# ishine/TTS-3

Hardware: AMD Instinct MI355X
Metric: audio samples/sec + RTF, HiFiGAN-v1 22.05kHz 80-mel, batch 32 @ 1/2/4/8 GPU (higher is better)
Workload: dtype fp32 (power-of-2 scaled fp16 hi/lo split on fp16 MFMA, fp32 accumulate); 1 GPU; HiFiGAN-v1 22.05kHz inference, [32,80,1024] mel per GPU (replicate pad 5), fp32; model=HiFiGAN-v1 (hifigan_config.py generator_model_params), global_batch=32, seq_len=1024, parallelism=dp1 (utterance sharding; no collectives)

## Files before the change

### tts-3_amd/csrc/conv_device.hpp

```cpp
#pragma once

#include "common.hpp"

namespace tts {

typedef __amdgpu_buffer_rsrc_t rsrc_t;
typedef unsigned u32x4_t __attribute__((ext_vector_type(4)));
typedef unsigned u32x2_t __attribute__((ext_vector_type(2)));
typedef float f32x2 __attribute__((ext_vector_type(2)));
constexpr unsigned OOB_OFF = 0x80000000u;

#ifndef ACT_ABLATE
#define ACT_ABLATE 0
#endif
__device__ __forceinline__ unsigned act_range(unsigned bytes) {
  return (ACT_ABLATE && bytes != 0xFFFFFFFFu && bytes > 65536u) ? 65536u : bytes;
}
__device__ __forceinline__ rsrc_t make_rsrc(const void* p, unsigned bytes) {
  return __builtin_amdgcn_make_buffer_rsrc(const_cast<void*>(p), (short)0, (int)act_range(bytes), 0x00020000);
}
__device__ __forceinline__ float bload(rsrc_t r, unsigned voff, unsigned soff) {
  return __builtin_bit_cast(float, __builtin_amdgcn_raw_buffer_load_b32(r, (int)voff, (int)soff, 0));
}
__device__ __forceinline__ f32x4 bload4(rsrc_t r, unsigned voff, unsigned soff) {
  return __builtin_bit_cast(f32x4, __builtin_amdgcn_raw_buffer_load_b128(r, (int)voff, (int)soff, 0));
}
#ifndef TTS_ST_POL
#define TTS_ST_POL 0
#endif
#ifndef TTS_LDX_POL
#define TTS_LDX_POL 0
#endif
template <int POL = TTS_LDX_POL>
__device__ __forceinline__ float bload_x(rsrc_t r, unsigned voff, unsigned soff) {
  return __builtin_bit_cast(float, __builtin_amdgcn_raw_buffer_load_b32(r, (int)voff, (int)soff, POL));
}
__device__ __forceinline__ void bstore(rsrc_t r, float v, unsigned voff, unsigned soff) {
  __builtin_amdgcn_raw_buffer_store_b32(__builtin_bit_cast(unsigned, v), r, (int)voff, (int)soff, TTS_ST_POL);
}
__device__ __forceinline__ unsigned short f32_to_bf16_bits(float v) {
  return __builtin_bit_cast(unsigned short, (__bf16)v);
}
__device__ __forceinline__ float bf16_bits_to_f32(unsigned b) { return __builtin_bit_cast(float, b << 16); }
__device__ __forceinline__ float bf16_round(float v) { return bf16_bits_to_f32(f32_to_bf16_bits(v)); }
template <bool B16>
struct PlaneT {
  static constexpr unsigned ES = 4u;
  __device__ static __forceinline__ float ld(rsrc_t r, unsigned voff, unsigned soff) { return bload(r, voff, soff); }
  __device__ static __forceinline__ void st(rsrc_t r, float v, unsigned voff, unsigned soff) { bstore(r, v, voff, soff); }
  __device__ static __forceinline__ float rt(float v) { return v; }
};
template <>
struct PlaneT<true> {
  static constexpr unsigned ES = 2u;
  __device__ static __forceinline__ float ld(rsrc_t r, unsigned voff, unsigned soff) {
    return bf16_bits_to_f32((unsigned)__builtin_amdgcn_raw_buffer_load_b16(r, (int)voff, (int)soff, 0));
  }
  __device__ static __forceinline__ void st(rsrc_t r, float v, unsigned voff, unsigned soff) {
    __builtin_amdgcn_raw_buffer_store_b16(f32_to_bf16_bits(v), r, (int)voff, (int)soff, TTS_ST_POL);
  }
  __device__ static __forceinline__ float rt(float v) { return bf16_round(v); }
};
template <bool B16>
__device__ __forceinline__ const void* plane_at(const float* p, size_t e) {
  return reinterpret_cast<const char*>(p) + e * PlaneT<B16>::ES;
}
template <bool B16>
__device__ __forceinline__ f32x4 pload4(rsrc_t r, unsigned voff, unsigned soff) {
  if constexpr (B16) {
    const u32x2_t w = __builtin_bit_cast(u32x2_t, __builtin_amdgcn_raw_buffer_load_b64(r, (int)voff, (int)soff, 0));
    return f32x4{bf16_bits_to_f32(w[0] & 0xffffu), bf16_bits_to_f32(w[0] >> 16), bf16_bits_to_f32(w[1] & 0xffffu),
                 bf16_bits_to_f32(w[1] >> 16)};
  } else {
    return bload4(r, voff, soff);
  }
}
template <bool B16>
__device__ __forceinline__ void pstore4(rsrc_t r, f32x4 v, unsigned voff, unsigned soff) {
  if constexpr (B16) {
    const u32x2_t w = {(unsigned)f32_to_bf16_bits(v[0]) | ((unsigned)f32_to_bf16_bits(v[1]) << 16),
                       (unsigned)f32_to_bf16_bits(v[2]) | ((unsigned)f32_to_bf16_bits(v[3]) << 16)};
    __builtin_amdgcn_raw_buffer_store_b64(__builtin_bit_cast(u32x2_t, w), r, (int)voff, (int)soff, TTS_ST_POL);
  } else {
    __builtin_amdgcn_raw_buffer_store_b128(__builtin_bit_cast(u32x4_t, v), r, (int)voff, (int)soff, TTS_ST_POL);
  }
}

__device__ __forceinline__ void lds_dma_b128(const void* base, unsigned bytes, unsigned voff, const void* lds) {
  const unsigned long long p = reinterpret_cast<unsigned long long>(base);
  const u32x4_t d = {(unsigned)__builtin_amdgcn_readfirstlane((int)(unsigned)p),
                     (unsigned)__builtin_amdgcn_readfirstlane((int)((unsigned)(p >> 32) & 0xffffu)),
                     (unsigned)__builtin_amdgcn_readfirstlane((int)act_range(bytes)), 0x00020000u};
  const unsigned m =
      (unsigned)__builtin_amdgcn_readfirstlane((int)(unsigned)(unsigned long)(__attribute__((address_space(3))) const void*)lds);
#pragma clang diagnostic push
#pragma clang diagnostic ignored "-Winline-asm"
  asm volatile("s_mov_b32 m0, %2\n\ts_nop 0\n\tbuffer_load_dwordx4 %0, %1, 0 offen lds" ::"v"(voff), "s"(d), "s"(m)
               : "memory", "m0");
#pragma clang diagnostic pop
}

__device__ __forceinline__ void l2_touch_dma(const void* base, unsigned bytes, unsigned voff, const void* lds) {
  const unsigned long long p = reinterpret_cast<unsigned long long>(base);
  const u32x4_t d = {(unsigned)__builtin_amdgcn_readfirstlane((int)(unsigned)p),
                     (unsigned)__builtin_amdgcn_readfirstlane((int)((unsigned)(p >> 32) & 0xffffu)),
                     (unsigned)__builtin_amdgcn_readfirstlane((int)act_range(bytes)), 0x00020000u};
  const unsigned m =
      (unsigned)__builtin_amdgcn_readfirstlane((int)(unsigned)(unsigned long)(__attribute__((address_space(3))) const void*)lds);
#pragma clang diagnostic push
#pragma clang diagnostic ignored "-Winline-asm"
  asm volatile("s_mov_b32 m0, %2\n\ts_nop 0\n\tbuffer_load_dword %0, %1, 0 offen lds" ::"v"(voff), "s"(d), "s"(m)
               : "memory", "m0");
#pragma clang diagnostic pop
}

__device__ __forceinline__ float lrelu2(float x, float slope) { return fmaxf(x, x * slope); }
__device__ __forceinline__ int wave_id() { return __builtin_amdgcn_readfirstlane((int)(threadIdx.x >> 6)); }

__device__ __forceinline__ int xlds_off(int g, int r, int q, int xrows) {
  return (g * xrows + r) * 8 + 4 * (q ^ ((r >> 3) & 1));
}

template <int CTRL, int ROWS>
__device__ __forceinline__ float dpp_max_step(float v) {
  const int o = __builtin_amdgcn_update_dpp(__builtin_bit_cast(int, v), __builtin_bit_cast(int, v), CTRL, ROWS, 0xF, false);
  return fmaxf(v, __builtin_bit_cast(float, o));
}
__device__ __forceinline__ float wave_max(float v) {
  v = dpp_max_step<0xB1, 0xF>(v);
  v = dpp_max_step<0x4E, 0xF>(v);
  v = dpp_max_step<0x141, 0xF>(v);
  v = dpp_max_step<0x140, 0xF>(v);
  v = dpp_max_step<0x142, 0xA>(v);
  v = dpp_max_step<0x143, 0xC>(v);
  return __builtin_bit_cast(float, __builtin_amdgcn_readlane(__builtin_bit_cast(int, v), 63));
}

__device__ __forceinline__ void publish_amax(unsigned* slots, int b, float v) {
  v = wave_max(v);
  if ((threadIdx.x & 63) == 0) atomicMax(slots + (size_t)b * 64 + (blockIdx.x & 63), __float_as_uint(v));
}

__device__ __forceinline__ void publish_amax_block(unsigned* slots, int b, float v) {
  __shared__ float red[4];
  v = wave_max(v);
  if ((threadIdx.x & 63) == 0) red[threadIdx.x >> 6] = v;
  __syncthreads();
  if (threadIdx.x == 0)
    atomicMax(slots + (size_t)b * 64 + (blockIdx.x & 63),
              __float_as_uint(fmaxf(fmaxf(red[0], red[1]), fmaxf(red[2], red[3]))));
}

template <int TM, int TN, bool RES, int ZM, bool AMAX, bool YB = false>
__device__ __forceinline__ void conv_epilogue_impl(const Conv1dArgs& a, const f32x16 (&acc)[TM][TN], int b,
                                                   int tbase, int cobase, int lane, int tend,
                                                   const float* sbias, int sbase) {
  using PY = PlaneT<YB>;
  const int half = lane >> 5;
  const int l32 = lane & 31;
  const int Cout = a.Cout;
  const int Tout = a.Tout;
  const unsigned plane = (unsigned)Cout * (unsigned)Tout * PY::ES;
  const size_t item = (size_t)b * (a.o_bstride ? a.o_bstride : (int64_t)Cout * Tout);
  const rsrc_t rres = make_rsrc(RES ? plane_at<YB>(a.res, item) : a.bias, RES ? plane : 0u);
  const rsrc_t rz = make_rsrc(ZM >= 2 ? plane_at<YB>(a.z, item) : a.bias, ZM >= 2 ? plane : 0u);
  const rsrc_t rout = make_rsrc(plane_at<YB>(a.zmode == 0 ? a.y : a.z, item), plane);
  const rsrc_t rcv = make_rsrc(a.cvec ? a.cvec + (size_t)b * (a.cvec_bstride ? a.cvec_bstride : (int64_t)Cout) : a.bias,
                               a.cvec ? (unsigned)Cout * 4u : 0u);
  const rsrc_t rmask = make_rsrc(a.mask ? a.mask + (size_t)b * Tout : a.bias, a.mask ? (unsigned)Tout * 4u : 0u);
  const rsrc_t rbias = make_rsrc(a.bias, (unsigned)Cout * 4u);
  const bool has_mask = a.mask != nullptr;
  const bool mask_res = RES && a.mask_res && has_mask;
  const float oslope = a.out_slope;
  const float zdiv = a.zdiv;
  const unsigned rowb = (unsigned)Tout * PY::ES;
  float vmax = 0.f;
#pragma unroll
  for (int m = 0; m < TM; ++m) {
    float bv[16];
#pragma unroll
    for (int r = 0; r < 16; ++r) {
      const unsigned co = (unsigned)(cobase + m * 32 + (r & 3) + 8 * (r >> 2) + 4 * half);
      bv[r] = sbias ? sbias[(int)co - sbase] : bload(rbias, co * 4u, 0u) + bload(rcv, co * 4u, 0u);
    }
#pragma unroll
    for (int n = 0; n < TN; ++n) {
      const int t = tbase + n * 32 + l32;
      const int row0 = cobase + m * 32 + 4 * half;
      const bool tok = t < Tout && t < tend;
      const unsigned voff = tok ? ((unsigned)row0 * (unsigned)Tout + (unsigned)t) * PY::ES : OOB_OFF;
      const float mv = has_mask ? bload(rmask, (tok ? (unsigned)t * 4u : OOB_OFF), 0u) : 1.f;
      const float mv2 = mask_res ? mv : 1.f;
      unsigned vo[16];
      float rv[16], zv[16];
// ... 190 lines not shown
```

### tts-3_amd/csrc/wino8_kernel.hpp

```cpp
#pragma once

#include <type_traits>

#include "wino_kernel.hpp"

namespace tts {

__device__ __forceinline__ void lds_sync() { asm volatile("s_waitcnt lgkmcnt(0)\n\ts_barrier" ::: "memory"); }

#ifndef WINO_STAMPS
#define WINO_STAMPS 0
#endif
#define WSTAMP(i)                                                                                            \
  do {                                                                                                       \
    if (WINO_STAMPS && (threadIdx.x & 63) == 0) {                                                            \
      const size_t wg = blockIdx.x + (size_t)gridDim.x * (blockIdx.y + (size_t)gridDim.y * blockIdx.z);      \
      reinterpret_cast<unsigned long long*>(a.z)[(wg * 8 + (threadIdx.x >> 6)) * 32 + (i)] =                   \
          __builtin_amdgcn_s_memtime();                                                                      \
    }                                                                                                        \
  } while (0)

template <class S, int K, int D, bool XB = false>
struct Wino8Cfg {
  static constexpr int ES = XB ? 2 : 4;
  static constexpr int AL = 16 / ES;
  static constexpr int NCH = wino_chunks(K);
  static constexpr int NS = kWinoPoints * NCH;
  static constexpr int PAD = D * (K - 1) / 2;
  static constexpr int BNT = 64;
  static constexpr int J = BNT / D;
  static constexpr int TW = 4 * D * J;
  static constexpr int XROWS = BNT + (NCH - 1) * D;
  static constexpr int PLANE = XROWS * S::ROWB;
  static constexpr int TSZ = kWinoPoints * PLANE;
  static constexpr bool RT_ROFF = XB && TW % 8 != 0;
  static constexpr int ROFF = RT_ROFF ? 7 : (AL - PAD % AL) % AL;
  static constexpr int RSPAN = (XROWS - 1) % D + 4 * D * ((XROWS - 1) / D) + 6 * D + ROFF + 1;
  static constexpr int RSPAN4 = (RSPAN + AL - 1) / AL * AL;
  static constexpr int RPITCH = RSPAN4 % (2 * AL) == AL ? RSPAN4 : RSPAN4 + AL;
  static constexpr int RF4 = (16 * RPITCH / AL + 63) / 64 * 64;
  static constexpr int RSZ = RF4 * 16;
  static constexpr int NDMA = RF4 / 64;
  static constexpr int UNITS = XROWS * 4;
  static constexpr int UPW = (UNITS + 7) / 8;
  static constexpr int PITCH = 256;
  static_assert(UPW <= 64 && UNITS <= 256 + 64 && 3 * NCH >= 3, "one transform round per wave; the DMA spreads over 3 steps");
  static_assert(2 * (UNITS - 256) <= 4 * 64, "spread leftover jobs: one per lane of waves 4-7");
  static_assert(TW <= PITCH, "");
  static constexpr int EPI = 4 * 16 * PITCH * 4 > 8 * 8 * 4 * 64 * 4 ? 4 * 16 * PITCH * 4 : 8 * 8 * 4 * 64 * 4;
  static constexpr int TSM = 2 * TSZ > EPI ? 2 * TSZ : EPI;
};

template <class S, int K, int D, bool LRELU, int PL = 0>
__global__ __launch_bounds__(512) void conv1d_wino8_kernel(Conv1dArgs a) {
  constexpr bool XB = (PL & kPlaneXB16) != 0, YB = (PL & kPlaneYB16) != 0;
  using C = Wino8Cfg<S, K, D, XB>;
  constexpr int NP = S::NP;
  constexpr int NCH = C::NCH;
  constexpr bool H3 = S::SCALED;
  static_assert(PL == 0 || !H3, "bf16 planes: the bf16 scheme only");
#ifndef WINO8_PD
#define WINO8_PD 3
#endif
#ifndef WINO8_EARLY_W
#define WINO8_EARLY_W 0
#endif
#ifndef WINO8_PD1
#define WINO8_PD1 4
#endif
#ifndef WINO8_PD11
#define WINO8_PD11 WINO8_PD
#endif
#ifndef WINO8_PD_B1
#define WINO8_PD_B1 3
#endif
#ifndef WINO8_PD1_B1
#define WINO8_PD1_B1 4
#endif
#ifndef WINO8_GAP7
#define WINO8_GAP7 1
#endif
#ifndef WINO8_GAP11
#define WINO8_GAP11 1
#endif
  __shared__ __attribute__((aligned(16))) unsigned char tsm[C::TSM];
  __shared__ __attribute__((aligned(16))) unsigned char rsm[2 * C::RSZ];
  __shared__ float wbias[128];

  const int tid = threadIdx.x;
  const int lane = tid & 63;
  const int wave = __builtin_amdgcn_readfirstlane(tid >> 6);
  const int wm = wave & 3;
  const int grp = wave >> 2;
  const int half = lane >> 5;
  const int l32 = lane & 31;
  const int bx = blockIdx.x, mt = blockIdx.y, b = blockIdx.z;
  const int t0 = bx * C::TW;
  const int Tin = a.Tin;
  const int Cin = a.Cin;
  const int nc = a.n_chunks;
  const int ex = H3 ? amax_exp(a.amax_in, b) + kWinoBtShift : 0;
  const float xscale = H3 ? ldexpf(1.f, -ex) : 1.f;
  const float slope = a.in_slope;
  const char* xb = static_cast<const char*>(plane_at<XB>(a.x, (size_t)b * (a.x_bstride ? a.x_bstride : (int64_t)Cin * Tin)));
  const unsigned chb = (unsigned)Tin * (unsigned)C::ES;

  const int roff = C::RT_ROFF ? (((t0 - C::PAD) % 8) + 8) % 8 : C::ROFF;
  const int ta = t0 - C::PAD - roff;
#ifndef WINO8_ASM_DMA
#define WINO8_ASM_DMA 1
#endif
  auto dma = [&](int c, int rb, int k0 = 0, int k1 = 64) {
    const int c0 = c * 16;
    const rsrc_t rx = make_rsrc(xb + (size_t)c0 * chb, (unsigned)(Cin - c0) * chb);
    for (int i = wm + 4 * k0; i < C::NDMA && i < wm + 4 * k1; i += 4) {
      const int f = i * 64 + lane;
      constexpr int UPR = C::RPITCH / C::AL;
      const int ch = f / UPR, t = ta + C::AL * (f - ch * UPR);
      const unsigned vo = (ch < 16 && t >= 0 && t < Tin) ? (unsigned)ch * chb + (unsigned)t * (unsigned)C::ES : OOB_OFF;
      if (WINO8_ASM_DMA) {
        lds_dma_b128(xb + (size_t)c0 * chb, (unsigned)(Cin - c0) * chb, vo, rsm + rb * C::RSZ + i * 1024);
      } else {
        __builtin_amdgcn_raw_ptr_buffer_load_lds(
            rx, (__attribute__((address_space(3))) void*)(rsm + rb * C::RSZ + i * 1024), 16, (int)vo, 0, 0, 0);
      }
    }
  };

#ifndef WINO8_DENSE
// ... 25 lines not shown
#ifndef WINO8_REMAT11
#define WINO8_REMAT11 1
#endif
  constexpr bool remat = K == 11 ? WINO8_REMAT11 : WINO8_REMAT;
  auto job_unit = [&](int& jrow, int& jq) {
    if (remat && WINO8_DENSE && grp == TG) {
      int ln;
      asm volatile("v_mbcnt_lo_u32_b32 %0, -1, 0\n\tv_mbcnt_hi_u32_b32 %0, -1, %0" : "=v"(ln));
      const int uu = wm * 64 + ln;
      jrow = uu >> 2;
      jq = uu & 3;
    } else {
      jrow = jrow0;
      jq = jq0;
    }
  };
  auto job_load = [&](int rb, int j) {
    if (SPREAD && grp != TG && j >= 2) return;
    if (!uok) return;
    int jrow, jq;
    job_unit(jrow, jq);
    if constexpr (D == 1 && XB) {
      const u32x2_t* raw8 =
          reinterpret_cast<const u32x2_t*>(rsm + rb * C::RSZ) + (4 * jq + piece(j)) * (C::RPITCH / 4) + jrow;
#pragma unroll
      for (int u4 = 0; u4 < NU; ++u4) jraw8[u4] = raw8[u4];
    } else if constexpr (D == 1) {
      const f32x4* raw4 =
          reinterpret_cast<const f32x4*>(rsm + rb * C::RSZ) + (4 * jq + piece(j)) * (C::RPITCH / 4) + jrow;
#pragma unroll
      for (int u4 = 0; u4 < NU; ++u4) jraw4[u4] = raw4[u4];
    } else if constexpr (XB) {
      const int jjj = jrow / D, jrho = jrow - jjj * D;
      const unsigned short* raw = reinterpret_cast<const unsigned short*>(rsm + rb * C::RSZ) +
                                  (4 * jq + piece(j)) * C::RPITCH + jrho + 4 * D * jjj + roff;
#pragma unroll
      for (int k = 0; k < 7; ++k) jraw[k] = bf16_bits_to_f32(raw[D * k]);
    } else {
      const int jjj = jrow / D, jrho = jrow - jjj * D;
      const float* raw = reinterpret_cast<const float*>(rsm + rb * C::RSZ) + (4 * jq + piece(j)) * C::RPITCH +
                         jrho + 4 * D * jjj + C::ROFF;
#pragma unroll
      for (int k = 0; k < 7; ++k) jraw[k] = raw[D * k];
    }
  };
  auto job_finish = [&](int tb, int j) {
    if (SPREAD && grp != TG && j >= 2) return;
    if (!uok) return;
    int jrow, jq;
    job_unit(jrow, jq);
    float v[7], t[7];
#pragma unroll
    for (int k = 0; k < 7; ++k) {
      float x;
      if constexpr (D == 1 && XB) {
        const unsigned w = jraw8[(C::ROFF + k) / 4][((C::ROFF + k) % 4) / 2];
        x = bf16_bits_to_f32((C::ROFF + k) % 2 ? w >> 16 : w & 0xffffu);
      } else {
        x = D == 1 ? jraw4[(C::ROFF + k) / 4][(C::ROFF + k) % 4] : jraw[k];
      }
      if (LRELU) x = lrelu2(x, slope);
      v[k] = H3 ? x * xscale : x;
    }
    wino_bt(v, t);
    if ((j & 1) == 0) {
#pragma unroll
      for (int k = 0; k < 7; ++k) tkeep[k] = t[k];
      return;
    }
    unsigned char* base = tsm + tb * C::TSZ + jrow * S::ROWB + 4 * jq + 16 * (piece(j) >> 1);
#pragma unroll
    for (int p = 0; p < kWinoPoints; ++p) {
      unsigned w[NP];
      split_pair<S>(tkeep[p], t[p], w);
#pragma unroll
      for (int q = 0; q < NP; ++q) *reinterpret_cast<unsigned*>(base + p * C::PLANE + 32 * q) = w[q];
    }
  };

  const int mb = mt * 4 + wm;
  const rsrc_t ra = make_rsrc(a.w + ((size_t)mb * nc * C::NS) * (NP * 256), 0xFFFFFFFFu);
  const unsigned avoff = (unsigned)lane * 16u;

#ifndef WINO8_NOXCH
#define WINO8_NOXCH 0
#endif
  constexpr bool NX = WINO8_NOXCH != 0;
  constexpr int NA = NX ? 7 : 4, NB = NX ? 1 : 2;
  f32x16 acc[NA][NB];
#pragma unroll
  for (int p = 0; p < NA; ++p)
#pragma unroll
    for (int n = 0; n < NB; ++n) acc[p][n] = f32x16{};
  WSTAMP(0);

  float bpre = 0.f;
  if (tid < 128) {
    const int co = mt * 128 + tid;
    if (co < a.Cout) {
      bpre = a.bias[co];
      const float cv = a.cvec ? a.cvec[(size_t)b * (a.cvec_bstride ? a.cvec_bstride : (int64_t)a.Cout) + co] : 0.f;
      bpre = bpre + cv;
    }
  }
  if (grp == 1) {
    dma(0, 0);
    if (nc > 1) dma(1, 1);
  }
  auto prologue = [&](auto wl_tag) {
    constexpr int WL = decltype(wl_tag)::value;
    if (grp == 1) {
      if (nc > 1) asm volatile("s_waitcnt vmcnt(%0)" ::"n"(C::NDMA / 4 + WL) : "memory");
      else asm volatile("s_waitcnt vmcnt(%0)" ::"n"(WL) : "memory");
    }
    WSTAMP(1);
    if (tid < 128) wbias[tid] = bpre;
    lds_sync();
#pragma unroll
    for (int j = 0; j < 4; ++j) {
      job_load(0, j);
      job_finish(0, j);
    }
    if (grp == 1) asm volatile("s_waitcnt vmcnt(0)" ::: "memory");
    lds_sync();
    WSTAMP(2);
  };
  if (!WINO8_EARLY_W) prologue(std::integral_constant<int, 0>{});

  auto run = [&](auto npg_tag, auto p0_tag, auto g1_tag) {
    constexpr int NPG = decltype(npg_tag)::value;
    constexpr int P0 = decltype(p0_tag)::value;
    constexpr bool G1 = decltype(g1_tag)::value;
    constexpr int NV = NPG * NCH;
    constexpr int PD = NP == 1 ? (G1 ? WINO8_PD1_B1 : WINO8_PD_B1)
                               : (G1 ? WINO8_PD1 : (K == 11 ? WINO8_PD11 : WINO8_PD));
    constexpr int GAP0 = K == 11 ? WINO8_GAP11 : WINO8_GAP7;
    constexpr int GAP = GAP0 < NV / 4 ? GAP0 : NV / 4;
    auto aoff = [&](int ck, int v) {
      const int ck2 = ck + v / NV, v2 = v % NV;
      return ck2 < nc ? (unsigned)((ck2 * C::NS + (v2 / NPG) * 7 + P0 + v2 % NPG) * NP) * 1024u : 0u;
    };
    f32x4 ar[PD + 1][NP], bcur[NB][NP], bnext[NB][NP];
#pragma unroll
    for (int v = 0; v < PD; ++v)
#pragma unroll
      for (int q = 0; q < NP; ++q) ar[v][q] = bload4(ra, avoff, aoff(0, v) + (unsigned)q * 1024u);
    if (WINO8_EARLY_W) prologue(std::integral_constant<int, PD * NP>{});
    auto read_b = [&](const unsigned char* tl, int v, f32x4 (*dst)[NP]) {
      const int p = P0 + v % NPG, c = v / NPG;
#pragma unroll
      for (int n = 0; n < NB; ++n) {
        const unsigned char* ptr = tl + p * C::PLANE + ((NX ? grp : n) * 32 + l32 + c * D) * S::ROWB + 16 * half;
#pragma unroll
        for (int q = 0; q < NP; ++q) dst[n][q] = *reinterpret_cast<const f32x4*>(ptr + 32 * q);
      }
    };
    for (int ck = 0; ck < nc; ++ck) {
      const int tb = ck & 1;
      const unsigned char* tl = tsm + tb * C::TSZ;
      const bool more = ck + 1 < nc;
      read_b(tl, 0, bcur);
      if (ck < 8) WSTAMP(3 + 2 * ck);
#pragma unroll
      for (int v = 0; v < NV; ++v) {
#pragma unroll
        for (int q = 0; q < NP; ++q)
          ar[PD][q] = (WINO_ABLATE & 4) ? ar[0][q]
                                        : bload4(ra, avoff, ((WINO_ABLATE & 64) ? 0u : aoff(ck, v + PD)) + (unsigned)q * 1024u);
        if (v + 1 < NV) read_b(tl, v + 1, bnext);
        if ((WINO_ABLATE & 32) == 0 && G1 && ck + 2 < nc && v < 3) dma(ck + 2, tb, 2 * v, v == 2 ? 64 : 2 * v + 2);
        __builtin_amdgcn_sched_barrier(0);
        const int p = v % NPG;
#pragma unroll
        for (int e = 0; e < S::NPROD; ++e)
#pragma unroll
          for (int n = 0; n < NB; ++n) {
            if (WINO_ABLATE & 8) acc[p][n][e] += ar[0][S::PA[e]][0] * bcur[n][S::PB[e]][0];
            else acc[p][n] = S::mfma(ar[0][S::PA[e]], bcur[n][S::PB[e]], acc[p][n]);
          }
#pragma unroll
        for (int pp = 0; pp < PD; ++pp)
#pragma unroll
          for (int q = 0; q < NP; ++q) ar[pp][q] = ar[pp + 1][q];
        if (v + 1 < NV) {
#pragma unroll
          for (int n = 0; n < NB; ++n)
#pragma unroll
            for (int q = 0; q < NP; ++q) bcur[n][q] = bnext[n][q];
        }
#pragma unroll
        for (int j = 0; j < 4; ++j) {
          const int vj = (j * NV) / 4;
          if ((WINO_ABLATE & 2) == 0 && more) {
            if (GAP > 0 && vj + GAP < NV && v == vj + GAP) job_finish(tb ^ 1, j);
            if (v == vj) {
              job_load(tb ^ 1, j);
              if (GAP == 0 || vj + GAP >= NV) job_finish(tb ^ 1, j);
            }
          }
        }
      }
      constexpr int NAFTER = (PD < NV - 3 ? PD : NV - 3) * NP;
      if (G1) asm volatile("s_waitcnt vmcnt(%0)" ::"n"(NAFTER) : "memory");
      if (ck < 8) WSTAMP(4 + 2 * ck);
      lds_sync();
    }
  };
#ifndef WINO8_PRIO
#define WINO8_PRIO 0
#endif
  if (WINO8_PRIO == 1 && grp == 1) __builtin_amdgcn_s_setprio(1);
  if (WINO8_PRIO == 2 && grp == 0) __builtin_amdgcn_s_setprio(1);
  if constexpr (NX) {
    if (grp == 0) run(std::integral_constant<int, 7>{}, std::integral_constant<int, 0>{}, std::false_type{});
    else run(std::integral_constant<int, 7>{}, std::integral_constant<int, 0>{}, std::true_type{});
  } else {
    if (grp == 0) run(std::integral_constant<int, 4>{}, std::integral_constant<int, 0>{}, std::false_type{});
    else run(std::integral_constant<int, 3>{}, std::integral_constant<int, 4>{}, std::true_type{});
  }

#ifndef WINO8_EPI_PF
#define WINO8_EPI_PF 0
#endif
  if constexpr (WINO8_EPI_PF && D == 1) {
    if (a.res || a.zmode >= 2) {
      constexpr unsigned YES = PlaneT<YB>::ES;
      constexpr int LPR = C::TW * (int)YES / 128;
      const unsigned plane = (unsigned)a.Cout * (unsigned)a.Tout * YES;
      const size_t item = (size_t)b * (a.o_bstride ? a.o_bstride : (int64_t)a.Cout * a.Tout);
      const void* pres = a.res ? plane_at<YB>(a.res, item) : nullptr;
      const void* pz = a.zmode >= 2 ? plane_at<YB>(a.z, item) : nullptr;
#pragma unroll
      for (int i = 0; i < (128 * LPR + 511) / 512; ++i) {
        const int l = tid + 512 * i;
        const int co = mt * 128 + l / LPR, ln = l % LPR;
        const int t = t0 + ln * (128 / (int)YES);
        const unsigned vo = (l < 128 * LPR && co < a.Cout && t < a.Tout) ? ((unsigned)co * (unsigned)a.Tout + (unsigned)t) * YES : OOB_OFF;
        if (pres) l2_touch_dma(pres, plane, vo, rsm);
        if (pz) l2_touch_dma(pz, plane, vo, rsm + 256);
      }
    }
  }

  if (WINO_ABLATE & 16) {
    float sum = 0.f;
#pragma unroll
    for (int p = 0; p < NA; ++p)
#pragma unroll
      for (int n = 0; n < NB; ++n)
#pragma unroll
        for (int r = 0; r < 16; ++r) sum += acc[p][n][r];
    if (sum == 1234.5f) a.y[threadIdx.x] = sum;
    return;
  }
  const float sc = H3 ? ldexpf(1.f, ex + a.w_exp) : 1.f;
  const int nk = grp;
  float y[4][16];
  if constexpr (NX) {
#pragma unroll
    for (int r = 0; r < 16; ++r) {
      const float m0 = acc[0][0][r], m1 = acc[1][0][r], m2 = acc[2][0][r], m3 = acc[3][0][r];
      const float m4 = acc[4][0][r], m5 = acc[5][0][r], m6 = acc[6][0][r];
      const float s12 = m1 + m2, d12 = m1 - m2;
      y[0][r] = ((m0 + s12) + m3) + (m4 + m5);
      y[1][r] = fmaf(2.f, m3, d12) + fmaf(-2.f, m4, 0.5f * m5);
      y[2][r] = fmaf(4.f, m3, s12) + fmaf(4.f, m4, 0.25f * m5);
      y[3][r] = fmaf(8.f, m3, d12) + (fmaf(-8.f, m4, 0.125f * m5) + m6);
    }
    WSTAMP(20);
  } else {
  float yp[2][4][16];
#pragma unroll
  for (int n = 0; n < 2; ++n)
#pragma unroll
    for (int r = 0; r < 16; ++r) {
      if (grp == 0) {
        const float m0 = acc[0][n][r], m1 = acc[1][n][r], m2 = acc[2][n][r], m3 = acc[3][n][r];
        const float s12 = m1 + m2, d12 = m1 - m2;
        yp[n][0][r] = (m0 + s12) + m3;
        yp[n][1][r] = fmaf(2.f, m3, d12);
        yp[n][2][r] = fmaf(4.f, m3, s12);
        yp[n][3][r] = fmaf(8.f, m3, d12);
      } else {
        const float m4 = acc[0][n][r], m5 = acc[1][n][r], m6 = acc[2][n][r];
        yp[n][0][r] = m4 + m5;
        yp[n][1][r] = fmaf(-2.f, m4, 0.5f * m5);
        yp[n][2][r] = fmaf(4.f, m4, 0.25f * m5);
        yp[n][3][r] = fmaf(-8.f, m4, 0.125f * m5) + m6;
      }
    }
  WSTAMP(20);
  f32x4* xch = reinterpret_cast<f32x4*>(tsm);
  lds_sync();
#pragma unroll
  for (int h = 0; h < 2; ++h) {
#pragma unroll
    for (int r = 0; r < 8; ++r) {
      f32x4 v;
#pragma unroll
      for (int i = 0; i < 4; ++i) v[i] = grp == 0 ? yp[1][i][8 * h + r] : yp[0][i][8 * h + r];
      xch[((wm * 2 + grp) * 8 + r) * 64 + lane] = v;
    }
    lds_sync();
#pragma unroll
    for (int r = 0; r < 8; ++r) {
      const f32x4 other = xch[((wm * 2 + (1 - grp)) * 8 + r) * 64 + lane];
#pragma unroll
      for (int i = 0; i < 4; ++i) y[i][8 * h + r] = (grp == 0 ? yp[0][i][8 * h + r] : yp[1][i][8 * h + r]) + other[i];
    }
    lds_sync();
  }
  }

  WSTAMP(21);
  const int zm = a.zmode <= 1 ? 0 : a.zmode;
  const int cobase = mt * 128 + wm * 32;
  auto finish = [&](auto res_tag, auto zm_tag) {
    constexpr bool RES = decltype(res_tag)::value;
    constexpr int ZM = decltype(zm_tag)::value;
    const int Cout = a.Cout;
    const int Tout = a.Tout;
    constexpr unsigned YES = PlaneT<YB>::ES;
    const unsigned plane = (unsigned)Cout * (unsigned)Tout * YES;
    const size_t item = (size_t)b * (a.o_bstride ? a.o_bstride : (int64_t)Cout * Tout);
    const rsrc_t rres = make_rsrc(RES ? plane_at<YB>(a.res, item) : a.bias, RES ? plane : 0u);
    const rsrc_t rz = make_rsrc(ZM >= 2 ? plane_at<YB>(a.z, item) : a.bias, ZM >= 2 ? plane : 0u);
    const rsrc_t rout = make_rsrc(plane_at<YB>(a.zmode == 0 ? a.y : a.z, item), plane);
    const float oslope = a.out_slope;
    const float zdiv = a.zdiv;
    float vmax = 0.f;
    if constexpr (D == 1) {
      const int t = t0 + 4 * (nk * 32 + l32);
      const int nvalid = Tout - t < 4 ? (Tout - t > 0 ? Tout - t : 0) : 4;
      const bool full = nvalid == 4 && (Tout & 3) == 0;
      constexpr int GR = (RES && ZM >= 2) ? 8 : 16;
#pragma unroll
      for (int r0 = 0; r0 < 16; r0 += GR) {
        float bias[GR];
        unsigned voff[GR];
        WinoIn gin[GR];
#pragma unroll
        for (int k = 0; k < GR; ++k) {
          const int r = r0 + k;
          const unsigned co = (unsigned)(cobase + (r & 3) + 8 * (r >> 2) + 4 * half);
          bias[k] = wbias[co - (unsigned)(mt * 128)];
          voff[k] = nvalid > 0 ? (co * (unsigned)Tout + (unsigned)t) * YES : OOB_OFF;
          gin[k] = wino_gather<RES, ZM, YB>(rres, rz, voff[k], full, nvalid);
        }
#pragma unroll
        for (int k = 0; k < GR; ++k) {
          const int r = r0 + k;
          const f32x4 yv = {y[0][r], y[1][r], y[2][r], y[3][r]};
          const f32x4 v = wino_apply<RES, ZM, H3>(yv, bias[k], oslope, zdiv, gin[k], nvalid, vmax, sc);
          wino_store<YB>(rout, v, voff[k], full, nvalid);
        }
      }
    } else {
      float* tile = reinterpret_cast<float*>(tsm) + wm * (16 * C::PITCH);
      const int nn = nk * 32 + l32;
      const int jj = nn / D, rho = nn - (nn / D) * D;
      const int tl = 4 * lane;
      const int t = t0 + tl;
      const int lim = (C::TW < Tout - t0 ? C::TW : Tout - t0) - tl;
      const int nvalid = lim < 4 ? (lim > 0 ? lim : 0) : 4;
      const bool full = nvalid == 4 && (Tout & 3) == 0;
#pragma unroll
      for (int ps = 0; ps < 2; ++ps) {
        if (jj < C::J) {
#pragma unroll
          for (int r = 8 * ps; r < 8 * ps + 8; ++r) {
            const int rl = (r & 3) + 8 * ((r >> 2) - 2 * ps) + 4 * half;
#pragma unroll
            for (int i = 0; i < 4; ++i) tile[rl * C::PITCH + rho + D * (4 * jj + i)] = y[i][r];
          }
        }
        lds_sync();
        float bias[8];
        unsigned voff[8];
        WinoIn gin[8];
#pragma unroll
        for (int rr = 0; rr < 8; ++rr) {
          const int co = cobase + 16 * ps + grp * 8 + rr;
          bias[rr] = wbias[co - mt * 128];
          voff[rr] = nvalid > 0 ? ((unsigned)co * (unsigned)Tout + (unsigned)t) * YES : OOB_OFF;
          gin[rr] = wino_gather<RES, ZM, YB>(rres, rz, voff[rr], full, nvalid);
        }
#pragma unroll
        for (int rr = 0; rr < 8; ++rr) {
          const f32x4 yv = *reinterpret_cast<const f32x4*>(tile + (grp * 8 + rr) * C::PITCH + tl);
          const f32x4 v = wino_apply<RES, ZM, H3>(yv, bias[rr], oslope, zdiv, gin[rr], nvalid, vmax, sc);
          wino_store<YB>(rout, v, voff[rr], full, nvalid);
        }
        lds_sync();
      }
// ... 76 lines not shown
```

### tts-3_amd/csrc/wino_kernel.hpp

```cpp
#pragma once

#include "split_device.hpp"
#include "wino_consts.hpp"

namespace tts {

#ifndef WINO_ABLATE
#define WINO_ABLATE 0
#endif


__host__ __device__ inline void wino_bt(const float (&v)[7], float (&t)[7]) {
  float p[6];
#pragma unroll
  for (int k = 0; k < 6; ++k) p[k] = fmaf(-2.f, v[k + 1], v[k]);
  const float A = fmaf(-4.f, p[1], p[3]);
  const float Bq = fmaf(-4.f, p[2], p[4]);
  const float Cq = p[1] - p[3];
  const float Dq = p[2] - p[4];
  t[0] = fmaf(4.f, p[0], fmaf(-5.f, p[2], p[4]));
  t[1] = A + Bq;
  t[2] = A - Bq;
  t[3] = fmaf(2.f, Cq, Dq);
  t[4] = fmaf(2.f, Cq, -Dq);
  t[5] = fmaf(4.f, v[1], fmaf(-5.f, v[3], v[5]));
  t[6] = fmaf(5.f, p[3], fmaf(-4.f, p[1], -p[5]));
}

__host__ __device__ inline void wino_at(const float (&m)[7], float (&y)[4]) {
  const float a = m[1] + m[2], b = m[1] - m[2], c = m[3] + m[4], e = m[3] - m[4];
  y[0] = ((m[0] + a) + c) + m[5];
  y[1] = fmaf(2.f, e, b) + 0.5f * m[5];
  y[2] = fmaf(4.f, c, a) + 0.25f * m[5];
  y[3] = (fmaf(8.f, e, b) + 0.125f * m[5]) + m[6];
}

template <class S>
__device__ __forceinline__ void split_pair(float x0, float x1, unsigned (&w)[S::NP]) {
  S::split2(x0, x1, w);
}

template <class S, int NCH, int D, int TN>
struct WinoCfg {
  static constexpr int NPT = kWinoPoints;
  static constexpr int NS = NPT * NCH;
  static constexpr int BNT = 32 * TN;
  static constexpr int J = BNT / D;
  static constexpr int TW = 4 * D * J;
  static constexpr int XROWS = BNT + (NCH - 1) * D;
  static constexpr int PLANE = XROWS * S::ROWB;
  static constexpr int XSZB = NPT * PLANE;
  static constexpr int UNITS = XROWS * 4;
  static constexpr int UPT = (UNITS + 255) / 256;
  static constexpr int NJOB = 2 * UPT;
  static constexpr int JS0 = NS * 3 / 7;
  static constexpr int JSTEP = (NS - JS0) / NJOB > 0 ? (NS - JS0) / NJOB : 1;
  static_assert(J >= 1, "tile narrower than the dilation");
  static constexpr int PITCH = TW <= 128 ? 128 : 256;
  static_assert(TW <= 256, "epilogue transpose: at most 256 samples per row");
  static constexpr int SMEM = 2 * XSZB > 4 * 16 * PITCH * 4 ? 2 * XSZB : 4 * 16 * PITCH * 4;
};

struct WinoIn {
  f32x4 rv, zv;
};
template <bool RES, int ZM, bool YB = false>
__device__ __forceinline__ WinoIn wino_gather(const rsrc_t& rres, const rsrc_t& rz, unsigned voff, bool full, int nvalid) {
  using PY = PlaneT<YB>;
  WinoIn g;
  g.rv = f32x4{};
  g.zv = f32x4{};
  if (full) {
    if (RES) g.rv = pload4<YB>(rres, voff, 0u);
    if (ZM >= 2) g.zv = pload4<YB>(rz, voff, 0u);
  } else {
#pragma unroll
    for (int j = 0; j < 4; ++j) {
      const unsigned o = j < nvalid ? voff + PY::ES * j : OOB_OFF;
      if (RES) g.rv[j] = PY::ld(rres, o, 0u);
      if (ZM >= 2) g.zv[j] = PY::ld(rz, o, 0u);
    }
  }
  return g;
}

template <bool RES, int ZM, bool H3>
__device__ __forceinline__ f32x4 wino_apply(f32x4 y, float bias, float oslope, float zdiv, const WinoIn& g, int nvalid,
                                             float& vm, float sc = 1.f) {
  f32x4 v;
#pragma unroll
  for (int j = 0; j < 4; ++j) {
    float x = lrelu2(fmaf(y[j], sc, bias), oslope);
    if (RES) x = x + g.rv[j];
    if (ZM == 2) x = g.zv[j] + x;
    if (ZM == 3) x = (g.zv[j] + x) / zdiv;
    if (H3 && j < nvalid) vm = fmaxf(vm, fabsf(x));
    v[j] = x;
  }
  return v;
}

template <bool YB = false>
__device__ __forceinline__ void wino_store(const rsrc_t& rout, f32x4 v, unsigned voff, bool full, int nvalid) {
  using PY = PlaneT<YB>;
  if (full) {
    pstore4<YB>(rout, v, voff, 0u);
  } else {
#pragma unroll
    for (int j = 0; j < 4; ++j) PY::st(rout, v[j], j < nvalid ? voff + PY::ES * j : OOB_OFF, 0u);
  }
}

template <class C, int TN, bool H3, bool RES, int ZM>
__device__ __forceinline__ void wino_epilogue(const Conv1dArgs& a, const f32x16 (&acc)[kWinoPoints][TN], float sc,
                                              int b, int t0, int cobase, int lane, unsigned char* lds) {
  constexpr int D = C::TW / (4 * C::J);
  const int half = lane >> 5;
  const int l32 = lane & 31;
  const int Cout = a.Cout;
  const int Tout = a.Tout;
  const unsigned plane = (unsigned)Cout * (unsigned)Tout * 4u;
  const size_t item = (size_t)b * (a.o_bstride ? a.o_bstride : (int64_t)Cout * Tout);
  const rsrc_t rres = make_rsrc(RES ? a.res + item : a.bias, RES ? plane : 0u);
  const rsrc_t rz = make_rsrc(ZM >= 2 ? a.z + item : a.bias, ZM >= 2 ? plane : 0u);
  const rsrc_t rout = make_rsrc((a.zmode == 0 ? a.y : a.z) + item, plane);
  const rsrc_t rbias = make_rsrc(a.bias, (unsigned)Cout * 4u);
  const rsrc_t rcv = make_rsrc(a.cvec ? a.cvec + (size_t)b * (a.cvec_bstride ? a.cvec_bstride : (int64_t)Cout) : a.bias,
                               a.cvec ? (unsigned)Cout * 4u : 0u);
// ... 128 lines not shown
    for (int k = 0; k < 7; ++k) {
      const int ts = tb + D * k;
      uvoff[i][k] = (u < C::UNITS && ts >= 0 && ts < Tin) ? (unsigned)(4 * q) * chb + (unsigned)ts * 4u : OOB_OFF;
    }
    ulds[i] = u < C::UNITS ? row * S::ROWB + 4 * q : -1;
  }

  float xr[C::UPT][4][7];
  auto load_x = [&](int c) {
    const int c0 = c * 16;
    const rsrc_t rx = make_rsrc(xb + (size_t)c0 * Tin, (unsigned)(Cin - c0) * chb);
#pragma unroll
    for (int i = 0; i < C::UPT; ++i)
#pragma unroll
      for (int j = 0; j < 4; ++j)
#pragma unroll
        for (int k = 0; k < 7; ++k) xr[i][j][k] = bload(rx, uvoff[i][k] + (unsigned)j * chb, 0u);
  };
  auto stage_job = [&](int buf, int i, int jp) {
    if (ulds[i] < 0) return;
    float t[2][7];
#pragma unroll
    for (int h = 0; h < 2; ++h) {
      float v[7];
#pragma unroll
      for (int k = 0; k < 7; ++k) {
        float x = xr[i][2 * jp + h][k];
        if (LRELU) x = lrelu2(x, slope);
        v[k] = H3 ? x * xscale : x;
      }
      wino_bt(v, t[h]);
    }
    unsigned char* base = smem + buf * C::XSZB + ulds[i] + 16 * jp;
#pragma unroll
    for (int p = 0; p < NPT; ++p) {
      unsigned w[NP];
      split_pair<S>(t[0][p], t[1][p], w);
#pragma unroll
      for (int q = 0; q < NP; ++q) *reinterpret_cast<unsigned*>(base + p * C::PLANE + 32 * q) = w[q];
    }
  };

  const int wmu = __builtin_amdgcn_readfirstlane(wm);
  const int mb = mt * 4 + wmu;
  const rsrc_t ra = make_rsrc(a.w + ((size_t)mb * nc * C::NS) * (NP * 256), 0xFFFFFFFFu);
  const unsigned avoff = (unsigned)lane * 16u;

  f32x16 acc[NPT][TN];
#pragma unroll
  for (int p = 0; p < NPT; ++p)
#pragma unroll
    for (int n = 0; n < TN; ++n) acc[p][n] = f32x16{};

  f32x4 ar[PD + 1][NP], bcur[TN][NP], bnext[TN][NP];
#pragma unroll
  for (int p = 0; p < PD; ++p)
#pragma unroll
    for (int q = 0; q < NP; ++q) ar[p][q] = bload4(ra, avoff, (unsigned)(p * NP + q) * 1024u);

  auto read_b = [&](const unsigned char* xl, int s, f32x4 (*dst)[NP]) {
    const int p = s % NPT, c = s / NPT;
#pragma unroll
    for (int n = 0; n < TN; ++n) {
      const unsigned char* ptr = xl + p * C::PLANE + (n * 32 + l32 + c * D) * S::ROWB + 16 * half;
#pragma unroll
      for (int q = 0; q < NP; ++q) dst[n][q] = *reinterpret_cast<const f32x4*>(ptr + 32 * q);
    }
  };

  load_x(0);
#pragma unroll
  for (int i = 0; i < C::UPT; ++i)
#pragma unroll
    for (int jp = 0; jp < 2; ++jp) stage_job(0, i, jp);
  __syncthreads();

  for (int c = 0; c < nc; ++c) {
    const int buf = c & 1;
    const unsigned char* xl = smem + buf * C::XSZB;
    const bool more = c + 1 < nc;
    if ((WINO_ABLATE & 1) == 0 && more) load_x(c + 1);
    read_b(xl, 0, bcur);
#pragma unroll
    for (int s = 0; s < C::NS; ++s) {
      const int sg = c * C::NS + s;
#pragma unroll
      for (int q = 0; q < NP; ++q) ar[PD][q] = (WINO_ABLATE & 4) ? ar[0][q] : bload4(ra, avoff, (unsigned)((sg + PD) * NP + q) * 1024u);
      if (s + 1 < C::NS) read_b(xl, s + 1, bnext);
      __builtin_amdgcn_sched_barrier(0);
      const int p = s % NPT;
#pragma unroll
      for (int e = 0; e < S::NPROD; ++e)
#pragma unroll
        for (int n = 0; n < TN; ++n) {
          if (WINO_ABLATE & 8) acc[p][n][e] += ar[0][S::PA[e]][0] * bcur[n][S::PB[e]][0];
          else acc[p][n] = S::mfma(ar[0][S::PA[e]], bcur[n][S::PB[e]], acc[p][n]);
        }
#pragma unroll
      for (int pp = 0; pp < PD; ++pp)
#pragma unroll
        for (int q = 0; q < NP; ++q) ar[pp][q] = ar[pp + 1][q];
      if (s + 1 < C::NS) {
#pragma unroll
        for (int n = 0; n < TN; ++n)
#pragma unroll
          for (int q = 0; q < NP; ++q) bcur[n][q] = bnext[n][q];
      }
#pragma unroll
      for (int jb = 0; jb < C::NJOB; ++jb) {
        const int js = C::JS0 + jb * C::JSTEP;
        if ((WINO_ABLATE & 2) == 0 && more && s == (js < C::NS ? js : C::NS - 1)) stage_job(buf ^ 1, jb >> 1, jb & 1);
      }
    }
    __syncthreads();
  }

  const float sc = H3 ? ldexpf(1.f, ex + a.w_exp) : 1.f;
  const int zm = a.zmode <= 1 ? 0 : a.zmode;
  if (WINO_ABLATE & 16) {
    float sum = 0.f;
#pragma unroll
    for (int p = 0; p < NPT; ++p)
#pragma unroll
      for (int n = 0; n < TN; ++n)
#pragma unroll
        for (int r = 0; r < 16; ++r) sum += acc[p][n][r];
    if (sum == 1234.5f) a.y[threadIdx.x] = sum;
    return;
  }
  if (a.res) {
    if (zm == 0) wino_epilogue<C, TN, H3, true, 0>(a, acc, sc, b, t0, mt * 128 + wm * 32, lane, smem);
    else if (zm == 2) wino_epilogue<C, TN, H3, true, 2>(a, acc, sc, b, t0, mt * 128 + wm * 32, lane, smem);
    else wino_epilogue<C, TN, H3, true, 3>(a, acc, sc, b, t0, mt * 128 + wm * 32, lane, smem);
  } else {
    if (zm == 0) wino_epilogue<C, TN, H3, false, 0>(a, acc, sc, b, t0, mt * 128 + wm * 32, lane, smem);
    else if (zm == 2) wino_epilogue<C, TN, H3, false, 2>(a, acc, sc, b, t0, mt * 128 + wm * 32, lane, smem);
    else wino_epilogue<C, TN, H3, false, 3>(a, acc, sc, b, t0, mt * 128 + wm * 32, lane, smem);
  }
}

namespace wino_detail {
#ifndef WINO_PD
#define WINO_PD 2
#endif
#ifndef WINO_TN
#define WINO_TN 1
#endif
template <class S, int NCH, int D>
void launch_wino_d(const Conv1dArgs& a, int B, hipStream_t s) {
  constexpr int TN = WINO_TN, PD = WINO_PD;
  using C = WinoCfg<S, NCH, D, TN>;
  const dim3 grid(ceil_div(a.Tout, C::TW), ceil_div(a.Cout, 128), B);
  if constexpr (D == 1) {
    if (a.in_slope == 1.f) {
      hipLaunchKernelGGL((conv1d_wino_kernel<S, NCH, D, TN, PD, false>), grid, dim3(256), 0, s, a);
      return;
    }
  }
  hipLaunchKernelGGL((conv1d_wino_kernel<S, NCH, D, TN, PD, true>), grid, dim3(256), 0, s, a);
}

template <class S, int NCH>
void launch_wino_k(const Conv1dArgs& a, int B, hipStream_t s) {
  switch (a.dil) {
    case 1: launch_wino_d<S, NCH, 1>(a, B, s); break;
    case 3: launch_wino_d<S, NCH, 3>(a, B, s); break;
    case 5: launch_wino_d<S, NCH, 5>(a, B, s); break;
    default: throw Error(3, "conv1d(winograd): dilation must be 1, 3 or 5");
  }
}

template <class S>
void launch_wino_s(const Conv1dArgs& a, int B, int K, hipStream_t s) {
  TTS_REQUIRE(a.mask == nullptr && a.ups == 0 && a.gate == 0 && a.rep_pad == 0 && a.Tin == a.Tout &&
                  a.pad == a.dil * (K - 1) / 2,
              1, "conv1d(winograd): unsupported arguments");
  switch (K) {
    case 3: launch_wino_k<S, 1>(a, B, s); break;
    case 7: launch_wino_k<S, 2>(a, B, s); break;
    case 11: launch_wino_k<S, 3>(a, B, s); break;
    default: throw Error(3, "conv1d(winograd): kernel size must be 3, 7 or 11");
  }
}
}

}
```

Before: 167.4 million samples/s.

## Skip always-zero Winograd point-6 product and rebalance wino8 point groups

```diff
diff --git a/tts-3_amd/csrc/conv_device.hpp b/tts-3_amd/csrc/conv_device.hpp
--- a/tts-3_amd/csrc/conv_device.hpp
+++ b/tts-3_amd/csrc/conv_device.hpp
@@ -96,20 +96,6 @@
 #pragma clang diagnostic push
 #pragma clang diagnostic ignored "-Winline-asm"
   asm volatile("s_mov_b32 m0, %2\n\ts_nop 0\n\tbuffer_load_dwordx4 %0, %1, 0 offen lds" ::"v"(voff), "s"(d), "s"(m)
-               : "memory", "m0");
-#pragma clang diagnostic pop
-}
-
-__device__ __forceinline__ void l2_touch_dma(const void* base, unsigned bytes, unsigned voff, const void* lds) {
-  const unsigned long long p = reinterpret_cast<unsigned long long>(base);
-  const u32x4_t d = {(unsigned)__builtin_amdgcn_readfirstlane((int)(unsigned)p),
-                     (unsigned)__builtin_amdgcn_readfirstlane((int)((unsigned)(p >> 32) & 0xffffu)),
-                     (unsigned)__builtin_amdgcn_readfirstlane((int)act_range(bytes)), 0x00020000u};
-  const unsigned m =
-      (unsigned)__builtin_amdgcn_readfirstlane((int)(unsigned)(unsigned long)(__attribute__((address_space(3))) const void*)lds);
-#pragma clang diagnostic push
-#pragma clang diagnostic ignored "-Winline-asm"
-  asm volatile("s_mov_b32 m0, %2\n\ts_nop 0\n\tbuffer_load_dword %0, %1, 0 offen lds" ::"v"(voff), "s"(d), "s"(m)
                : "memory", "m0");
 #pragma clang diagnostic pop
 }
diff --git a/tts-3_amd/csrc/wino8_kernel.hpp b/tts-3_amd/csrc/wino8_kernel.hpp
--- a/tts-3_amd/csrc/wino8_kernel.hpp
+++ b/tts-3_amd/csrc/wino8_kernel.hpp
@@ -5,6 +5,11 @@
 #include "wino_kernel.hpp"
 
 namespace tts {
+
+__host__ __device__ constexpr int wino8_npg(int g) { return g == 0 ? 4 : 3; }
+__host__ __device__ constexpr int wino8_point(int g, int i) {
+  return g == 0 ? (i < 3 ? i + 1 : 6) : (i == 0 ? 0 : i + 3);
+}
 
 __device__ __forceinline__ void lds_sync() { asm volatile("s_waitcnt lgkmcnt(0)\n\ts_barrier" ::: "memory"); }
 
@@ -44,7 +49,7 @@
   static constexpr int UNITS = XROWS * 4;
   static constexpr int UPW = (UNITS + 7) / 8;
   static constexpr int PITCH = 256;
-  static_assert(UPW <= 64 && UNITS <= 256 + 64 && 3 * NCH >= 3, "one transform round per wave; the DMA spreads over 3 steps");
+  static_assert(UPW <= 64 && UNITS <= 256 + 64, "one transform round per wave");
   static_assert(2 * (UNITS - 256) <= 4 * 64, "spread leftover jobs: one per lane of waves 4-7");
   static_assert(TW <= PITCH, "");
   static constexpr int EPI = 4 * 16 * PITCH * 4 > 8 * 8 * 4 * 64 * 4 ? 4 * 16 * PITCH * 4 : 8 * 8 * 4 * 64 * 4;
@@ -236,11 +241,7 @@
   const rsrc_t ra = make_rsrc(a.w + ((size_t)mb * nc * C::NS) * (NP * 256), 0xFFFFFFFFu);
   const unsigned avoff = (unsigned)lane * 16u;
 
-#ifndef WINO8_NOXCH
-#define WINO8_NOXCH 0
-#endif
-  constexpr bool NX = WINO8_NOXCH != 0;
-  constexpr int NA = NX ? 7 : 4, NB = NX ? 1 : 2;
+  constexpr int NA = 4, NB = 2;
   f32x16 acc[NA][NB];
 #pragma unroll
   for (int p = 0; p < NA; ++p)
@@ -281,18 +282,20 @@
   };
   if (!WINO8_EARLY_W) prologue(std::integral_constant<int, 0>{});
 
-  auto run = [&](auto npg_tag, auto p0_tag, auto g1_tag) {
-    constexpr int NPG = decltype(npg_tag)::value;
-    constexpr int P0 = decltype(p0_tag)::value;
-    constexpr bool G1 = decltype(g1_tag)::value;
-    constexpr int NV = NPG * NCH;
+  auto run = [&](auto g_tag) {
+    constexpr int G = decltype(g_tag)::value;
+    constexpr int NPG = wino8_npg(G);
+    constexpr bool G1 = G == 1;
+    constexpr int ZS = (K % 4 == 3 && wino8_point(G, NPG - 1) == 6) ? 1 : 0;
+    constexpr int NV = NPG * NCH - ZS;
+    constexpr int NDS = NV < 3 ? NV : 3;
     constexpr int PD = NP == 1 ? (G1 ? WINO8_PD1_B1 : WINO8_PD_B1)
                                : (G1 ? WINO8_PD1 : (K == 11 ? WINO8_PD11 : WINO8_PD));
     constexpr int GAP0 = K == 11 ? WINO8_GAP11 : WINO8_GAP7;
     constexpr int GAP = GAP0 < NV / 4 ? GAP0 : NV / 4;
     auto aoff = [&](int ck, int v) {
       const int ck2 = ck + v / NV, v2 = v % NV;
-      return ck2 < nc ? (unsigned)((ck2 * C::NS + (v2 / NPG) * 7 + P0 + v2 % NPG) * NP) * 1024u : 0u;
+      return ck2 < nc ? (unsigned)((ck2 * C::NS + (v2 / NPG) * 7 + wino8_point(G, v2 % NPG)) * NP) * 1024u : 0u;
     };
     f32x4 ar[PD + 1][NP], bcur[NB][NP], bnext[NB][NP];
 #pragma unroll
@@ -301,10 +304,10 @@
       for (int q = 0; q < NP; ++q) ar[v][q] = bload4(ra, avoff, aoff(0, v) + (unsigned)q * 1024u);
     if (WINO8_EARLY_W) prologue(std::integral_constant<int, PD * NP>{});
     auto read_b = [&](const unsigned char* tl, int v, f32x4 (*dst)[NP]) {
-      const int p = P0 + v % NPG, c = v / NPG;
+      const int p = wino8_point(G, v % NPG), c = v / NPG;
 #pragma unroll
       for (int n = 0; n < NB; ++n) {
-        const unsigned char* ptr = tl + p * C::PLANE + ((NX ? grp : n) * 32 + l32 + c * D) * S::ROWB + 16 * half;
+        const unsigned char* ptr = tl + p * C::PLANE + (n * 32 + l32 + c * D) * S::ROWB + 16 * half;
 #pragma unroll
         for (int q = 0; q < NP; ++q) dst[n][q] = *reinterpret_cast<const f32x4*>(ptr + 32 * q);
       }
@@ -322,7 +325,7 @@
           ar[PD][q] = (WINO_ABLATE & 4) ? ar[0][q]
                                         : bload4(ra, avoff, ((WINO_ABLATE & 64) ? 0u : aoff(ck, v + PD)) + (unsigned)q * 1024u);
         if (v + 1 < NV) read_b(tl, v + 1, bnext);
-        if ((WINO_ABLATE & 32) == 0 && G1 && ck + 2 < nc && v < 3) dma(ck + 2, tb, 2 * v, v == 2 ? 64 : 2 * v + 2);
+        if ((WINO_ABLATE & 32) == 0 && G1 && ck + 2 < nc && v < NDS) dma(ck + 2, tb, 2 * v, v == NDS - 1 ? 64 : 2 * v + 2);
         __builtin_amdgcn_sched_barrier(0);
         const int p = v % NPG;
 #pragma unroll
@@ -354,47 +357,14 @@
           }
         }
       }
-      constexpr int NAFTER = (PD < NV - 3 ? PD : NV - 3) * NP;
+      constexpr int NAFTER = (PD < NV - NDS ? PD : NV - NDS) * NP;
       if (G1) asm volatile("s_waitcnt vmcnt(%0)" ::"n"(NAFTER) : "memory");
       if (ck < 8) WSTAMP(4 + 2 * ck);
       lds_sync();
     }
   };
-#ifndef WINO8_PRIO
-#define WINO8_PRIO 0
-#endif
-  if (WINO8_PRIO == 1 && grp == 1) __builtin_amdgcn_s_setprio(1);
-  if (WINO8_PRIO == 2 && grp == 0) __builtin_amdgcn_s_setprio(1);
-  if constexpr (NX) {
-    if (grp == 0) run(std::integral_constant<int, 7>{}, std::integral_constant<int, 0>{}, std::false_type{});
-    else run(std::integral_constant<int, 7>{}, std::integral_constant<int, 0>{}, std::true_type{});
-  } else {
-    if (grp == 0) run(std::integral_constant<int, 4>{}, std::integral_constant<int, 0>{}, std::false_type{});
-    else run(std::integral_constant<int, 3>{}, std::integral_constant<int, 4>{}, std::true_type{});
-  }
-
-#ifndef WINO8_EPI_PF
-#define WINO8_EPI_PF 0
-#endif
-  if constexpr (WINO8_EPI_PF && D == 1) {
-    if (a.res || a.zmode >= 2) {
-      constexpr unsigned YES = PlaneT<YB>::ES;
-      constexpr int LPR = C::TW * (int)YES / 128;
-      const unsigned plane = (unsigned)a.Cout * (unsigned)a.Tout * YES;
-      const size_t item = (size_t)b * (a.o_bstride ? a.o_bstride : (int64_t)a.Cout * a.Tout);
-      const void* pres = a.res ? plane_at<YB>(a.res, item) : nullptr;
-      const void* pz = a.zmode >= 2 ? plane_at<YB>(a.z, item) : nullptr;
-#pragma unroll
-      for (int i = 0; i < (128 * LPR + 511) / 512; ++i) {
-        const int l = tid + 512 * i;
-        const int co = mt * 128 + l / LPR, ln = l % LPR;
-        const int t = t0 + ln * (128 / (int)YES);
-        const unsigned vo = (l < 128 * LPR && co < a.Cout && t < a.Tout) ? ((unsigned)co * (unsigned)a.Tout + (unsigned)t) * YES : OOB_OFF;
-        if (pres) l2_touch_dma(pres, plane, vo, rsm);
-        if (pz) l2_touch_dma(pz, plane, vo, rsm + 256);
-      }
-    }
-  }
+  if (grp == 0) run(std::integral_constant<int, 0>{});
+  else run(std::integral_constant<int, 1>{});
 
   if (WINO_ABLATE & 16) {
     float sum = 0.f;
@@ -410,37 +380,24 @@
   const float sc = H3 ? ldexpf(1.f, ex + a.w_exp) : 1.f;
   const int nk = grp;
   float y[4][16];
-  if constexpr (NX) {
-#pragma unroll
-    for (int r = 0; r < 16; ++r) {
-      const float m0 = acc[0][0][r], m1 = acc[1][0][r], m2 = acc[2][0][r], m3 = acc[3][0][r];
-      const float m4 = acc[4][0][r], m5 = acc[5][0][r], m6 = acc[6][0][r];
-      const float s12 = m1 + m2, d12 = m1 - m2;
-      y[0][r] = ((m0 + s12) + m3) + (m4 + m5);
-      y[1][r] = fmaf(2.f, m3, d12) + fmaf(-2.f, m4, 0.5f * m5);
-      y[2][r] = fmaf(4.f, m3, s12) + fmaf(4.f, m4, 0.25f * m5);
-      y[3][r] = fmaf(8.f, m3, d12) + (fmaf(-8.f, m4, 0.125f * m5) + m6);
-    }
-    WSTAMP(20);
-  } else {
   float yp[2][4][16];
 #pragma unroll
   for (int n = 0; n < 2; ++n)
 #pragma unroll
     for (int r = 0; r < 16; ++r) {
       if (grp == 0) {
-        const float m0 = acc[0][n][r], m1 = acc[1][n][r], m2 = acc[2][n][r], m3 = acc[3][n][r];
+        const float m1 = acc[0][n][r], m2 = acc[1][n][r], m3 = acc[2][n][r], m6 = acc[3][n][r];
         const float s12 = m1 + m2, d12 = m1 - m2;
-        yp[n][0][r] = (m0 + s12) + m3;
+        yp[n][0][r] = s12 + m3;
         yp[n][1][r] = fmaf(2.f, m3, d12);
         yp[n][2][r] = fmaf(4.f, m3, s12);
-        yp[n][3][r] = fmaf(8.f, m3, d12);
+        yp[n][3][r] = fmaf(8.f, m3, d12) + m6;
       } else {
-        const float m4 = acc[0][n][r], m5 = acc[1][n][r], m6 = acc[2][n][r];
-        yp[n][0][r] = m4 + m5;
+        const float m0 = acc[0][n][r], m4 = acc[1][n][r], m5 = acc[2][n][r];
+        yp[n][0][r] = m0 + (m4 + m5);
         yp[n][1][r] = fmaf(-2.f, m4, 0.5f * m5);
         yp[n][2][r] = fmaf(4.f, m4, 0.25f * m5);
-        yp[n][3][r] = fmaf(-8.f, m4, 0.125f * m5) + m6;
+        yp[n][3][r] = fmaf(-8.f, m4, 0.125f * m5);
       }
     }
   WSTAMP(20);
@@ -463,7 +420,6 @@
       for (int i = 0; i < 4; ++i) y[i][8 * h + r] = (grp == 0 ? yp[0][i][8 * h + r] : yp[1][i][8 * h + r]) + other[i];
     }
     lds_sync();
-  }
   }
 
   WSTAMP(21);
diff --git a/tts-3_amd/csrc/wino_kernel.hpp b/tts-3_amd/csrc/wino_kernel.hpp
--- a/tts-3_amd/csrc/wino_kernel.hpp
+++ b/tts-3_amd/csrc/wino_kernel.hpp
@@ -28,11 +28,11 @@
 }
 
 __host__ __device__ inline void wino_at(const float (&m)[7], float (&y)[4]) {
-  const float a = m[1] + m[2], b = m[1] - m[2], c = m[3] + m[4], e = m[3] - m[4];
-  y[0] = ((m[0] + a) + c) + m[5];
-  y[1] = fmaf(2.f, e, b) + 0.5f * m[5];
-  y[2] = fmaf(4.f, c, a) + 0.25f * m[5];
-  y[3] = (fmaf(8.f, e, b) + 0.125f * m[5]) + m[6];
+  const float a = m[1] + m[2], b = m[1] - m[2];
+  y[0] = (a + m[3]) + (m[0] + (m[4] + m[5]));
+  y[1] = fmaf(2.f, m[3], b) + fmaf(-2.f, m[4], 0.5f * m[5]);
+  y[2] = fmaf(4.f, m[3], a) + fmaf(4.f, m[4], 0.25f * m[5]);
+  y[3] = (fmaf(8.f, m[3], b) + m[6]) + fmaf(-8.f, m[4], 0.125f * m[5]);
 }
 
 template <class S>
@@ -44,6 +44,7 @@
 struct WinoCfg {
   static constexpr int NPT = kWinoPoints;
   static constexpr int NS = NPT * NCH;
+  static constexpr int NSR = NS - 1;
   static constexpr int BNT = 32 * TN;
   static constexpr int J = BNT / D;
   static constexpr int TW = 4 * D * J;
@@ -338,11 +339,12 @@
     if ((WINO_ABLATE & 1) == 0 && more) load_x(c + 1);
     read_b(xl, 0, bcur);
 #pragma unroll
-    for (int s = 0; s < C::NS; ++s) {
-      const int sg = c * C::NS + s;
-#pragma unroll
-      for (int q = 0; q < NP; ++q) ar[PD][q] = (WINO_ABLATE & 4) ? ar[0][q] : bload4(ra, avoff, (unsigned)((sg + PD) * NP + q) * 1024u);
-      if (s + 1 < C::NS) read_b(xl, s + 1, bnext);
+    for (int s = 0; s < C::NSR; ++s) {
+      const int cpf = c + (s + PD) / C::NSR;
+      const int sg = cpf < nc ? cpf * C::NS + (s + PD) % C::NSR : 0;
+#pragma unroll
+      for (int q = 0; q < NP; ++q) ar[PD][q] = (WINO_ABLATE & 4) ? ar[0][q] : bload4(ra, avoff, (unsigned)(sg * NP + q) * 1024u);
+      if (s + 1 < C::NSR) read_b(xl, s + 1, bnext);
       __builtin_amdgcn_sched_barrier(0);
       const int p = s % NPT;
 #pragma unroll
@@ -356,7 +358,7 @@
       for (int pp = 0; pp < PD; ++pp)
 #pragma unroll
         for (int q = 0; q < NP; ++q) ar[pp][q] = ar[pp + 1][q];
-      if (s + 1 < C::NS) {
+      if (s + 1 < C::NSR) {
 #pragma unroll
         for (int n = 0; n < TN; ++n)
 #pragma unroll
@@ -365,7 +367,7 @@
 #pragma unroll
       for (int jb = 0; jb < C::NJOB; ++jb) {
         const int js = C::JS0 + jb * C::JSTEP;
-        if ((WINO_ABLATE & 2) == 0 && more && s == (js < C::NS ? js : C::NS - 1)) stage_job(buf ^ 1, jb >> 1, jb & 1);
+        if ((WINO_ABLATE & 2) == 0 && more && s == (js < C::NSR ? js : C::NSR - 1)) stage_job(buf ^ 1, jb >> 1, jb & 1);
       }
     }
     __syncthreads();
```

New measurement: 168.9 million samples/s (median of 6 runs). About the same (+0.9%).
